# tsy935/eeg-gnn-ssl

Hardware: AMD Instinct MI355X
Metric: EEG clips/sec (60s, 19ch, K=2, 2-layer x64) fwd+bwd (higher is better)
Workload: dtype f32

## Files before the change

eeg_gnn_ssl_amd/csrc/api.cpp:

```cpp
#include <atomic>
#include <cmath>
#include <cstdarg>
#include <cstdio>
#include <cstring>

#include <string>
#include <vector>

#include "../../include/eeg_dcrnn.h"
#include "../../include/eeg_dcrnn_dev.h"
#include "../../include/eeg_dcrnn_prof.h"
#include "kernels_decoder.h"
#include "kernels_diffuse.h"
#include "kernels_eval.h"
#include "kernels_data.h"
#include "kernels_feat.h"
#include "kernels_gemm.h"
#include "kernels_gemm_bf.h"
#include "kernels_graph.h"
#include "kernels_head.h"
#include "kernels_pack.h"
#include "spec_common.h"
#include "spec_launch.h"
#include "kernels_tail.h"
// ... 320 lines not shown
    return w;
}


int cell_weight_grads(const eeg_layer_dims* d, const float* X, const float* planes, size_t x_stride, const float* Hprev,
                      const float* RHs, const float* dXW, const float* P, const float* hpl_in, const float* rpl_in,
                      size_t h_stride, float* hpl_ws, float* rpl_ws, float* part, const BwdWs& w, bool accumulate,
                      float* dWg, float* dWc, hipStream_t st, BtMap bt = BtMap(), const float* bias_part = nullptr,
                      float* dbg = nullptr, float* dbc = nullptr) {
    const int S = d->T * d->B, R = S * d->N, H = d->H, M = d->M, Fin = d->Fin, N = d->N;
    const int acc = accumulate ? 8 : 0;
    SegPtrs sx;
    for (int m = 0; m < kMaxM; ++m) sx.p[m] = m == 0 ? X : (m < M ? planes + (size_t)(m - 1) * x_stride : nullptr);
    float* part_g = part + (w.part_g - w.partial);
    float* part_c = part + (w.part_c - w.partial);
    if (gemm_tn(w.tx, w.cx, sx, dXW, 3 * H, 0, part, st, "gemm_tn_x", bt)) return 1;
    const float* hpl = hpl_in;
    size_t hs = h_stride;
    if (hpl == nullptr) {
        if (diffuse_fwd(Hprev, P, d->p_batched, S, d->B, N, H, M, hpl_ws, st)) return 1;
        hpl = hpl_ws;
        hs = (size_t)R * H;
    }
    SegPtrs sh;
    for (int m = 0; m < kMaxM; ++m) sh.p[m] = m == 0 ? Hprev : (m < M ? hpl + (size_t)(m - 1) * hs : nullptr);
    const float* rpl = rpl_in;
    size_t rs = h_stride;
    if (rpl == nullptr) {
        if (diffuse_fwd(RHs, P, d->p_batched, S, d->B, N, H, M, rpl_ws, st)) return 1;
        rpl = rpl_ws;
        rs = (size_t)R * H;
    }
    SegPtrs sr;
    for (int m = 0; m < kMaxM; ++m) sr.p[m] = m == 0 ? RHs : (m < M ? rpl + (size_t)(m - 1) * rs : nullptr);
    if (w.pair) {
        if (launch_tnq_pair(w.thg.q, w.thc.q, sh, sr, M, H, R, dXW, 3 * H, 0, 2 * H, part_g, 2 * H, H, part_c, st, "gemm_tn_h"))
            return fail("gemm_tnq_pair: launch failed");
    } else {
        if (gemm_tn(w.thg, w.chg, sh, dXW, 3 * H, 0, part_g, st, "gemm_tn_hg")) return 1;
        if (gemm_tn(w.thc, w.chc, sr, dXW, 3 * H, 2 * H, part_c, st, "gemm_tn_hc")) return 1;
    }
    ReduceJobs jobs;
    const int Ks[3] = {M * Fin, M * H, M * H}, Os[3] = {3 * H, 2 * H, H}, ns[3] = {w.tx.nsplit, w.thg.nsplit, w.thc.nsplit};
    const float* parts[3] = {part, part_g, part_c};
    int nblocks = 0;
    for (int j = 0; j < 3; ++j) {
        jobs.part[j] = parts[j]; jobs.nsplit[j] = ns[j]; jobs.K[j] = Ks[j]; jobs.O[j] = Os[j];
        jobs.nblocks[j] = ceil_div(Ks[j] * Os[j], 64);
        nblocks += jobs.nblocks[j];
    }
    jobs.bias_part = bias_part; jobs.bias_B = d->B; jobs.dbg = dbg; jobs.dbc = dbc;
    if (bias_part != nullptr) nblocks += ceil_div(3 * H, 16);
    EEG_LAUNCH_P("reduce_unpack", reduce_unpack3_kernel, dim3(nblocks), dim3(256), 256 * sizeof(float4), st, jobs, acc, Fin, H, M, dWg, dWc);
    return check_launch("reduce_unpack");
}

size_t xs_spec(const eeg_layer_dims* d) { return d->x_plane_stride > 0 ? (size_t)d->x_plane_stride : 0; }
int cell_weight_grads_spectral(const eeg_layer_dims* d, const float* Xh, size_t x_gs, const float* hh, size_t hh_gs, const float* rhh,
                               const float* dYh, float* part, const BwdWs& w, float* dWg, float* dWc, hipStream_t st,
                               const float* bias_part, float* dbg, float* dbc) {
    const int S = d->T * d->B, H = d->H, M = d->M, Fin = d->Fin, N = d->N, Sp = spec_rows(S);
    float* part_g = part + (w.part_g - w.partial);
    float* part_c = part + (w.part_c - w.partial);
    const SpecTnPlan& g = w.gs;
    if (spec_plan_error("weight gradients (spectral)", g.error)) return 1;
    if (g.fused) {
        if (launch_tnf(g, Xh, x_gs, Fin, hh, hh_gs, rhh, dYh, Sp, N, part, part_g, part_c, st, "gemm_tn_f")) return fail("gemm_tnf: launch failed");
    } else {
        if (launch_tng(g, Xh, x_gs, Fin, Sp, N, dYh, part, st, "gemm_tn_x")) return fail("gemm_tng: launch failed");
        if (launch_tng_pair(g, hh, hh_gs, rhh, Sp, N, dYh, part_g, part_c, st, "gemm_tn_h")) return fail("gemm_tng_pair: launch failed");
    }
    ReduceJobs jobs{};
    SpecFoldJobs sj{};
    sj.basis = d->spectral; sj.N = N;
    sj.j[0] = SpecFoldJob{part, g.spg_x, Fin, 3 * H, ceil_div(Fin * 3 * H, 64)};
    sj.j[1] = SpecFoldJob{part_g, g.spg_h, H, 2 * H, ceil_div(H * 2 * H, 64)};
    sj.j[2] = SpecFoldJob{part_c, g.spg_h, H, H, ceil_div(H * H, 64)};
    int nblocks = sj.j[0].nblocks + sj.j[1].nblocks + sj.j[2].nblocks;
    jobs.bias_part = bias_part; jobs.bias_B = d->B; jobs.dbg = dbg; jobs.dbc = dbc;
    if (bias_part != nullptr) nblocks += ceil_div(3 * H, 16);
    const int ns_max = N * (g.spg_x > g.spg_h ? g.spg_x : g.spg_h);
    const size_t fold_lds = spec_fold_lds_bytes(M, ns_max);
    EEG_SET_MAX_LDS(reduce_unpack3s_kernel, fold_lds);
    EEG_LAUNCH_P("reduce_unpack", reduce_unpack3s_kernel, dim3(nblocks), dim3(256), fold_lds, st, jobs, sj, 0, Fin, H, M, dWg, dWc);
    return check_launch("reduce_unpack (spectral)");
}

int colsum_rows_per_chunk(int R) { int rpc = ceil_div(R, 512); return rpc < 64 ? 64 : rpc; }
size_t colsum_ws(int R, int C) { return (size_t)ceil_div(R, colsum_rows_per_chunk(R)) * C; }
int colsum(const float* A, int R, int C, int split, float* ws, float* out0, float* out1, hipStream_t st) {
    const int rpc = colsum_rows_per_chunk(R), nchunk = ceil_div(R, rpc);
    if (C % 4 == 0 && C <= 1024) {
        const int nrs = 256 / (C / 4);
        EEG_LAUNCH_P("reduce_bias", colsum_partial4_kernel, dim3(nchunk), dim3(256), (size_t)nrs * C * sizeof(float), st, A, R, C, rpc, ws);
    } else {
        EEG_LAUNCH_P("reduce_bias", colsum_partial_kernel, dim3(nchunk, ceil_div(C, 128)), dim3(256), 256 * sizeof(float), st, A, R, C, rpc, ws);
    }
    if (check_launch("colsum_partial")) return 1;
    EEG_LAUNCH_P("reduce_bias", colsum_final_kernel, dim3(ceil_div(C, 128)), dim3(128), 0, st, ws, nchunk, C, split, out0, out1);
    return check_launch("colsum_final");
}

struct DecLayout {
    size_t xin, proj_pack, proj_bias, hd, saved_total;
    size_t planes[8], hext[8], rs[8], us[8], cs[8], rhs[8], hpl[8], rpl[8];
    size_t dxw[8], dbias[8], dotot, da, dhn, z, partial, projt_pack, colsum, bwd_total;
    TnCall cp;
    TnPlan tp;
    BwdWs lw[8];
    eeg_layer_dims ld[8];
};
size_t align64(size_t v) { return (v + 63) / 64 * 64; }
DecLayout dec_layout(const eeg_decoder_dims* d) {
    DecLayout y;
    const size_t state = (size_t)d->B * d->N * d->H, R = (size_t)d->T * d->B * d->N;
    const int nct_o = ceil_div(d->Dout, 16), nct_h = ceil_div(d->H, 16);
    size_t o = 0;
    y.xin = o;       o += align64(R * d->Dout);
    y.proj_pack = o; o += align64((size_t)(d->H / 4) * nct_o * 64);
    y.proj_bias = o; o += align64((size_t)nct_o * 16);
    for (int l = 0; l < d->L; ++l) {
        const int fin = l == 0 ? d->Dout : d->H;
        y.ld[l] = eeg_layer_dims{d->T, d->B, d->N, d->H, fin, d->M, d->act, d->p_batched, 0, 0, 0};
        y.planes[l] = o; if (l == 0) o += align64((size_t)(d->M - 1) * R * fin);
        y.hext[l] = o;   o += align64((size_t)(d->T + 1) * state);
        y.rs[l] = o;     o += align64((size_t)d->T * state);
        y.us[l] = o;     o += align64((size_t)d->T * state);
        y.cs[l] = o;     o += align64((size_t)d->T * state);
        y.rhs[l] = o;    o += align64((size_t)d->T * state);
        y.hpl[l] = o;    o += align64((size_t)(d->M - 1) * (d->T + 1) * state);
        y.rpl[l] = o;    o += align64((size_t)(d->M - 1) * (d->T + 1) * state);
    }
    y.hd = d->dropout_p > 0.f ? o : y.hext[d->L - 1] + state;
    if (d->dropout_p > 0.f) o += align64((size_t)d->T * state);
    y.saved_total = o;
    o = 0;
    size_t part = 0;
    for (int l = 0; l < d->L; ++l) {
        y.lw[l] = bwd_ws(&y.ld[l], 0);
        y.dxw[l] = o; o += align64(R * 3 * d->H);
        const size_t pl = y.lw[l].total - y.lw[l].partial;
        part = pl > part ? pl : part;
    }
    for (int l = 0; l < d->L; ++l) { y.dbias[l] = o; o += (size_t)d->T * d->B * 3 * d->H; }
    o = align64(o);
    y.dotot = o;  o += align64(R * d->Dout);
    y.da = o;     o += align64(state);
    y.dhn = o;    o += align64(2 * (size_t)d->L * state);
    y.z = o;      o += align64((size_t)d->B * d->N * d->M * (d->Dout > d->H ? d->Dout : d->H));
    y.cp = tn_call(1, d->Dout, (int)R, d->H);
    y.tp = gemm_tn_plan(y.cp);
    const size_t pp = (size_t)y.tp.nsplit * d->Dout * d->H;
    part = pp > part ? pp : part;
    y.partial = o; o += align64(part);
    y.projt_pack = o; o += align64((size_t)(d->Dout / 4) * nct_h * 64);
    const size_t c1 = colsum_ws((int)R, d->Dout), c2 = colsum_ws(d->L * d->T * d->B, 3 * d->H);
    y.colsum = o; o += align64(c1 > c2 ? c1 : c2);
    y.bwd_total = o;
    return y;
}
int check_dropout_p(const char* who, float p) {
    if (!(p >= 0.f && p <= 1.f)) return fail("%s: dropout probability has to be between 0 and 1, but got %g", who, p);
    return 0;
}
int check_decoder_dims(const eeg_decoder_dims* d) {
    if (d->L < 1 || d->L > 8) return fail("decoder: num_rnn_layers=%d unsupported (1..8)", d->L);
    if (d->T < 1 || d->B < 1) return fail("decoder: empty sequence/batch (T=%d, B=%d)", d->T, d->B);
// ... 1306 lines not shown
```

eeg_gnn_ssl_amd/csrc/kernels_pack.h:

```cpp
#pragma once
#include "common.h"
#include "nnq_order.h"
#include "spec_common.h"
#include "pack_cell.h"

namespace eeg {

__global__ void pack_cell_kernel(const float* __restrict__ Wg, const float* __restrict__ bg,
                                 const float* __restrict__ Wc, const float* __restrict__ bc,
                                 float* __restrict__ out, CellPack p) {
    pack_cell_body(Wg, bg, Wc, bc, out, p, (int)blockIdx.x, (int)gridDim.x);
}

__global__ void pack_dense_kernel(const float* __restrict__ W, int F, int M, int O, float* __restrict__ out) {
    const size_t total = (size_t)F * M * O;
    const int nct = O / 16;
    for (size_t e = (size_t)blockIdx.x * blockDim.x + threadIdx.x; e < total; e += (size_t)gridDim.x * blockDim.x) {
        const int lane = e & 63, ct = (e >> 6) % nct, ks = (e >> 6) / nct;
        const int k = 4 * ks + (lane >> 4), j = 16 * ct + (lane & 15);
        const int m = k / F, f = k % F;
        out[e] = W[((size_t)f * M + m) * O + j];
    }
}

__global__ void pack_dense_t_kernel(const float* __restrict__ W, int F, int M, int O, float* __restrict__ out) {
    const int nct = round_up(M * F, 16) / 16;
    const size_t total = (size_t)(O / 4) * nct * 64;
    for (size_t e = (size_t)blockIdx.x * blockDim.x + threadIdx.x; e < total; e += (size_t)gridDim.x * blockDim.x) {
        const int lane = e & 63, ct = (e >> 6) % nct, ks = (e >> 6) / nct;
        const int o = 4 * ks + (lane >> 4), j = 16 * ct + (lane & 15);
        float v = 0.f;
        if (j < M * F) v = W[((size_t)(j % F) * M + j / F) * O + o];
        out[e] = v;
    }
}

__global__ void pack_linear_kernel(const float* __restrict__ W, int Out, int In, int transposed, float* __restrict__ out) {
    const int K = transposed ? In : Out, O = transposed ? Out : In;
    const int nct = (O + 15) / 16;
    const size_t total = (size_t)(K / 4) * nct * 64;
    for (size_t e = (size_t)blockIdx.x * blockDim.x + threadIdx.x; e < total; e += (size_t)gridDim.x * blockDim.x) {
        const int lane = e & 63, ct = (e >> 6) % nct, ks = (e >> 6) / nct;
        const int k = 4 * ks + (lane >> 4), j = 16 * ct + (lane & 15);
        float v = 0.f;
        if (j < O) v = transposed ? W[(size_t)j * In + k] : W[(size_t)k * In + j];
        out[e] = v;
    }
}

__device__ __forceinline__ void reduce_unpack_block(int block, const float* __restrict__ part, int nsplit, int K, int O,
                                                    int kind_flags, int Fin, int H, int M,
                                                    float* __restrict__ dWg, float* __restrict__ dWc) {
    EEG_DYN_SMEM(sm);
    float4 (*red)[16] = reinterpret_cast<float4 (*)[16]>(sm);
    const size_t total = (size_t)K * O;
    const int g = threadIdx.x >> 4, q = threadIdx.x & 15;
    const size_t idx4 = ((size_t)block * 16 + q) * 4;
    float4 a = make_float4(0.f, 0.f, 0.f, 0.f);
    if (idx4 < total) {
        for (int sp = g; sp < nsplit; sp += 16) {
            const float4 v = *reinterpret_cast<const float4*>(part + (size_t)sp * total + idx4);
            a.x += v.x; a.y += v.y; a.z += v.z; a.w += v.w;
        }
    }
    red[g][q] = a;
    __syncthreads();
    if (g != 0 || idx4 >= total) return;
    float4 sum = red[0][q];
#pragma unroll
    for (int u = 1; u < 16; ++u) {
        const float4 v = red[u][q];
        sum.x += v.x; sum.y += v.y; sum.z += v.z; sum.w += v.w;
    }
    const float sv[4] = {sum.x, sum.y, sum.z, sum.w};
    const bool accumulate = (kind_flags & 8) != 0;
    const int kind = kind_flags & 7;
#pragma unroll
    for (int e = 0; e < 4; ++e) {
        const size_t idx = idx4 + e;
        const int k = idx / O, o = idx % O;
        float* dst;
        if (kind == 0) {
            const int m = k / Fin, f = k % Fin;
            dst = o < 2 * H ? &dWg[((size_t)f * M + m) * (2 * H) + o] : &dWc[((size_t)f * M + m) * H + (o - 2 * H)];
        } else if (kind == 1) {
            dst = &dWg[((size_t)(Fin + k % H) * M + k / H) * (2 * H) + o];
        } else if (kind == 3) {
            dst = &dWg[idx];
        } else if (kind == 4) {
            dst = &dWg[((size_t)(k % Fin) * M + k / Fin) * O + o];
        } else {
            dst = &dWc[((size_t)(Fin + k % H) * M + k / H) * H + o];
        }
        *dst = accumulate ? *dst + sv[e] : sv[e];
    }
}
__global__ __launch_bounds__(256) void reduce_unpack_kernel(const float* __restrict__ part, int nsplit, int K, int O,
                                                            int kind_flags, int Fin, int H, int M,
                                                            float* __restrict__ dWg, float* __restrict__ dWc) {
    reduce_unpack_block(blockIdx.x, part, nsplit, K, O, kind_flags, Fin, H, M, dWg, dWc);
}
__device__ __forceinline__ void reduce_bias_block(int blk, float* sm, const float* __restrict__ part, int B, int H,
                                                  float* __restrict__ dbg, float* __restrict__ dbc) {
    const int c = threadIdx.x & 15, q = threadIdx.x >> 4;
    const int j = blk * 16 + c;
    float s = 0.f;
    if (j < 3 * H)
        for (int b = q; b < B; b += 16) s += part[(size_t)b * 3 * H + j];
    sm[q * 16 + c] = s;
    __syncthreads();
    if (q == 0 && j < 3 * H) {
        float t = 0.f;
        for (int i = 0; i < 16; ++i) t += sm[i * 16 + c];
        if (j < 2 * H) dbg[j] = t; else dbc[j - 2 * H] = t;
    }
}
struct ReduceJobs {
    const float* part[3]; int nsplit[3]; int K[3]; int O[3]; int nblocks[3];
    const float* bias_part; int bias_B; float* dbg; float* dbc;
};
__global__ __launch_bounds__(256) void reduce_unpack3_kernel(ReduceJobs jobs, int flags, int Fin, int H, int M,
                                                             float* __restrict__ dWg, float* __restrict__ dWc) {
    int b = blockIdx.x, j = 0;
    if (b >= jobs.nblocks[0]) { b -= jobs.nblocks[0]; j = 1; }
    if (j == 1 && b >= jobs.nblocks[1]) { b -= jobs.nblocks[1]; j = 2; }
    if (j == 2 && b >= jobs.nblocks[2]) {
        EEG_DYN_SMEM(sm);
        reduce_bias_block(b - jobs.nblocks[2], sm, jobs.bias_part, jobs.bias_B, H, jobs.dbg, jobs.dbc);
        return;
    }
    reduce_unpack_block(b, jobs.part[j], jobs.nsplit[j], jobs.K[j], jobs.O[j], j | flags, Fin, H, M, dWg, dWc);
}

__global__ __launch_bounds__(256) void reduce_unpack3s_kernel(ReduceJobs jobs, SpecFoldJobs sj, int flags, int Fin, int H, int M,
                                                              float* __restrict__ dWg, float* __restrict__ dWc) {
    int b = blockIdx.x;
#pragma unroll
    for (int k = 0; k < 3; ++k) {
        if (sj.j[k].part == nullptr) continue;
        if (b < sj.j[k].nblocks) {
            spec_fold_block(b, sj.j[k], k, sj.basis, sj.N, (flags & 8) != 0 ? 1 : 0, Fin, H, M, dWg, dWc);
            return;
        }
        b -= sj.j[k].nblocks;
    }
#pragma unroll
    for (int j = 1; j < 3; ++j) {
        if (sj.j[j].part != nullptr) continue;
        if (b < jobs.nblocks[j]) {
            reduce_unpack_block(b, jobs.part[j], jobs.nsplit[j], jobs.K[j], jobs.O[j], j | flags, Fin, H, M, dWg, dWc);
            return;
        }
        b -= jobs.nblocks[j];
    }
    EEG_DYN_SMEM(sm);
    reduce_bias_block(b, sm, jobs.bias_part, jobs.bias_B, H, jobs.dbg, jobs.dbc);
}

__global__ void colsum_partial_kernel(const float* __restrict__ A, int R, int C, int rpc, float* __restrict__ partial) {
    EEG_DYN_SMEM(sm);
    const int c = threadIdx.x & 127, q = threadIdx.x >> 7;
    const int col = blockIdx.y * 128 + c;
    const int r0 = blockIdx.x * rpc, r1 = (r0 + rpc < R) ? r0 + rpc : R;
    float a0 = 0.f, a1 = 0.f, a2 = 0.f, a3 = 0.f;
    if (col < C) {
        int r = r0 + q;
        for (; r + 6 < r1; r += 8) {
            a0 += A[(size_t)r * C + col];
            a1 += A[(size_t)(r + 2) * C + col];
            a2 += A[(size_t)(r + 4) * C + col];
            a3 += A[(size_t)(r + 6) * C + col];
        }
        for (; r < r1; r += 2) a0 += A[(size_t)r * C + col];
    }
    sm[q * 128 + c] = (a0 + a1) + (a2 + a3);
    __syncthreads();
    if (q == 0 && col < C) partial[(size_t)blockIdx.x * C + col] = sm[c] + sm[128 + c];
}
__global__ __launch_bounds__(256) void colsum_partial4_kernel(const float* __restrict__ A, int R, int C, int rpc,
                                                              float* __restrict__ partial) {
    EEG_DYN_SMEM(sm);
    const int c4n = C / 4, nrs = 256 / c4n;
    const int cq = threadIdx.x % c4n, q = threadIdx.x / c4n;
    const int r0 = blockIdx.x * rpc, r1 = (r0 + rpc < R) ? r0 + rpc : R;
    f32x4 a0 = {0.f, 0.f, 0.f, 0.f}, a1 = a0, a2 = a0, a3 = a0;
    if (q < nrs) {
        const float* p = A + 4 * cq;
        int r = r0 + q;
        for (; r + 3 * nrs < r1; r += 4 * nrs) {
            a0 += ld4(p + (size_t)r * C);
            a1 += ld4(p + (size_t)(r + nrs) * C);
            a2 += ld4(p + (size_t)(r + 2 * nrs) * C);
            a3 += ld4(p + (size_t)(r + 3 * nrs) * C);
        }
        for (; r < r1; r += nrs) a0 += ld4(p + (size_t)r * C);
        st4(sm + q * C + 4 * cq, (a0 + a1) + (a2 + a3));
    }
    __syncthreads();
    for (int col = threadIdx.x; col < C; col += 256) {
        float s = 0.f;
        for (int i = 0; i < nrs; ++i) s += sm[i * C + col];
        partial[(size_t)blockIdx.x * C + col] = s;
    }
}
__global__ void colsum_final_kernel(const float* __restrict__ partial, int nchunk, int C, int split,
                                    float* __restrict__ out0, float* __restrict__ out1) {
    const int col = blockIdx.x * blockDim.x + threadIdx.x;
    if (col >= C) return;
    float a0 = 0.f, a1 = 0.f, a2 = 0.f, a3 = 0.f;
    int i = 0;
    for (; i + 4 <= nchunk; i += 4) {
        a0 += partial[(size_t)i * C + col];
        a1 += partial[(size_t)(i + 1) * C + col];
        a2 += partial[(size_t)(i + 2) * C + col];
        a3 += partial[(size_t)(i + 3) * C + col];
    }
    for (; i < nchunk; ++i) a0 += partial[(size_t)i * C + col];
    const float s = (a0 + a1) + (a2 + a3);
// ... 50 lines not shown
```

eeg_gnn_ssl_amd/csrc/kernels_spectral.h:

```cpp
#pragma once
#include "spec_common.h"
#include "spec_launch.h"

namespace eeg {

__global__ __launch_bounds__(256) void spectral_basis_kernel(const float* __restrict__ S, int N, float* __restrict__ out) {
    EEG_DYN_SMEM(sm);
    double* A = reinterpret_cast<double*>(sm);
    double* V = A + 32 * 32;
    double* cs = V + 32 * 32;
    int* pq = reinterpret_cast<int*>(cs + 32);
    double* red = reinterpret_cast<double*>(pq + 32);
    const int tid = threadIdx.x;
    const int NP = (N + 1) & ~1, NH = NP / 2;
    for (int e = tid; e < 32 * 32; e += 256) {
        const int i = e >> 5, j = e & 31;
        A[e] = (i < N && j < N) ? 0.5 * ((double)S[i * N + j] + (double)S[j * N + i]) : 0.0;
        V[e] = i == j ? 1.0 : 0.0;
    }
    __syncthreads();
    for (int sweep = 0; sweep < kSpecSweeps; ++sweep) {
        for (int r = 0; r < NP - 1; ++r) {
            if (tid < NH) {
                int p = tid == 0 ? NP - 1 : (r + tid) % (NP - 1);
// ... 38 lines not shown
    }
    for (int e = tid; e < N * N; e += 256) out[e] = (float)V[(e / N) * 32 + (e % N)];
    for (int e = tid; e < kSpecTc; e += 256) {
        const int m = e >> 5, i = e & 31;
        double t = 0.0;
        if (i < N) {
            const double lam = A[i * 32 + i];
            double t0 = 1.0, t1 = lam;
            t = m == 0 ? t0 : t1;
            for (int k = 2; k <= m; ++k) { t = 2.0 * lam * t1 - t0; t0 = t1; t1 = t; }
        }
        out[N * N + e] = (float)t;
    }
    double rmax = 0.0, omax = 0.0, smax = 0.0;
    for (int e = tid; e < N * N; e += 256) {
        const int i = e / N, j = e % N;
        double rec = 0.0;
        for (int k = 0; k < N; ++k) rec += V[i * 32 + k] * A[k * 32 + k] * V[j * 32 + k];
        rmax = fmax(rmax, fabs((double)S[e] - rec));
        if (i != j) omax = fmax(omax, fabs(A[i * 32 + j]));
        smax = fmax(smax, fabs((double)S[e]));
    }
    for (int which = 0; which < 3; ++which) {
        __syncthreads();
        red[tid] = which == 0 ? rmax : (which == 1 ? omax : smax);
        __syncthreads();
        if (tid == 0) {
            double m = 0.0;
            for (int i = 0; i < 256; ++i) m = fmax(m, red[i]);
            out[N * N + kSpecTc + which] = (float)m;
        }
    }
    if (tid >= 3 && tid < kSpecInfo) out[N * N + kSpecTc + tid] = 0.f;
    if (tid < 32) {
        double c = 0.0;
        if (tid < N)
            for (int n = 0; n < N; ++n) c += V[n * 32 + tid];
        out[N * N + kSpecTc + kSpecInfo + tid] = (float)c;
    }
}

__device__ __forceinline__ void pack_spectral_body(const float* __restrict__ Wg, const float* __restrict__ Wc, const float* __restrict__ basis,
                                                   float* __restrict__ out, const SpecPack& p, int bid, int nb) {
    const int Fin = p.Fin, H = p.H, M = p.M, N = p.N;
    const float* tc = basis + N * N;
    const NnqOrder ox = make_nnq_order(1, Fin), ot = make_nnq_order(1, 3 * H);
    const size_t stride = (size_t)nb * blockDim.x;
    for (size_t idx = (size_t)bid * blockDim.x + threadIdx.x; idx < p.total; idx += stride) {
        if (idx >= p.sxr) {
            const size_t e0 = idx - p.sxr;
            const int i = (int)(e0 / p.sxr_stride), e = (int)(e0 - (size_t)i * p.sxr_stride), f = e / (3 * H), o = e - f * 3 * H;
            float v = 0.f;
            if (f < Fin)
                for (int m = 0; m < M; ++m) {
                    const float w = o < 2 * H ? Wg[((size_t)f * M + m) * (2 * H) + o] : Wc[((size_t)f * M + m) * H + (o - 2 * H)];
                    v = fmaf(tc[m * 32 + i], w, v);
                }
            out[idx] = v;
            continue;
        }
        const bool tr = idx >= p.sxtq;
        const size_t bs = tr ? p.sxtq_stride : p.sxq_stride, e0 = idx - (tr ? p.sxtq : p.sxq);
        const int i = (int)(e0 / bs);
        const size_t e = e0 - (size_t)i * bs;
        const int s4 = e & 3, lane = (e >> 2) & 63, nct = tr ? p.nct_t : p.nct_x;
        const int ct = (int)((e >> 8) % nct), c = (int)((e >> 8) / nct), j = 16 * ct + (lane & 15);
        const int k = nnq_k_of(tr ? ot : ox, c, lane >> 4, s4);
        float v = 0.f;
        if (k >= 0) {
            const int f = tr ? j : k, o = tr ? k : j;
            if (f < Fin) {
                for (int m = 0; m < M; ++m) {
                    const float w = o < 2 * H ? Wg[((size_t)f * M + m) * (2 * H) + o] : Wc[((size_t)f * M + m) * H + (o - 2 * H)];
                    v = fmaf(tc[m * 32 + i], w, v);
                }
            }
        }
        out[idx] = v;
    }
}
__global__ void pack_spectral_kernel(const float* __restrict__ Wg, const float* __restrict__ Wc, const float* __restrict__ basis,
                                     float* __restrict__ out, SpecPack p) {
    pack_spectral_body(Wg, Wc, basis, out, p, (int)blockIdx.x, (int)gridDim.x);
}

__device__ __forceinline__ size_t spec_sample(size_t r, int map, int T, int B) { return map ? (r % B) * (size_t)T + r / B : r; }

template <int N>
__global__ __launch_bounds__(256) void spec_mix_in_kernel(const float* __restrict__ X, const float* __restrict__ basis, int S, int Sp,
                                                         int F, int map, int T, int B, float* __restrict__ Xh) {
    const int F4 = F / 4, SPW = blockDim.x / F4;
    const int tl = threadIdx.x / F4, c4 = threadIdx.x % F4;
    if (tl >= SPW) return;
    const float* __restrict__ U = basis;
    const float4* X4 = reinterpret_cast<const float4*>(X);
    float4* O4 = reinterpret_cast<float4*>(Xh);
    for (int r = blockIdx.x * SPW + tl; r < Sp; r += gridDim.x * SPW) {
        if (r >= S) {
#pragma unroll
            for (int i = 0; i < N; ++i) O4[((size_t)i * Sp + r) * F4 + c4] = make_float4(0.f, 0.f, 0.f, 0.f);
            continue;
        }
        const size_t s = spec_sample((size_t)r, map, T, B);
        float4 x[N];
#pragma unroll
        for (int n = 0; n < N; ++n) x[n] = X4[(s * N + n) * F4 + c4];
#pragma unroll
        for (int i = 0; i < N; ++i) {
            float4 a = make_float4(0.f, 0.f, 0.f, 0.f);
#pragma unroll
            for (int n = 0; n < N; ++n) {
                const float u = U[n * N + i];
                a.x = fmaf(u, x[n].x, a.x);
                a.y = fmaf(u, x[n].y, a.y);
                a.z = fmaf(u, x[n].z, a.z);
                a.w = fmaf(u, x[n].w, a.w);
            }
            O4[((size_t)i * Sp + r) * F4 + c4] = a;
        }
    }
}

template <int N>
__global__ __launch_bounds__(256) void spec_mix_out_kernel(const float* __restrict__ Yh, const float* __restrict__ basis,
                                                          const float* __restrict__ bias, int S, int Sp, int F, int map, int T, int B,
                                                          float* __restrict__ Y) {
    const int F4 = F / 4, SPW = blockDim.x / F4;
    const int tl = threadIdx.x / F4, c4 = threadIdx.x % F4;
    if (tl >= SPW) return;
    const float* __restrict__ U = basis;
    const float4* I4 = reinterpret_cast<const float4*>(Yh);
    float4* O4 = reinterpret_cast<float4*>(Y);
    float4 bv = make_float4(0.f, 0.f, 0.f, 0.f);
    if (bias != nullptr) bv = reinterpret_cast<const float4*>(bias)[c4];
    for (int r = blockIdx.x * SPW + tl; r < S; r += gridDim.x * SPW) {
        const size_t s = spec_sample((size_t)r, map, T, B);
        float4 y[N];
#pragma unroll
        for (int i = 0; i < N; ++i) y[i] = I4[((size_t)i * Sp + r) * F4 + c4];
#pragma unroll
        for (int j = 0; j < N; ++j) {
            float4 a = bv;
#pragma unroll
            for (int i = 0; i < N; ++i) {
                const float u = U[j * N + i];
                a.x = fmaf(u, y[i].x, a.x);
                a.y = fmaf(u, y[i].y, a.y);
                a.z = fmaf(u, y[i].z, a.z);
                a.w = fmaf(u, y[i].w, a.w);
            }
            O4[(s * N + j) * F4 + c4] = a;
        }
    }
}

template <int DIR, int KS>
__global__ __launch_bounds__(256) void spec_mix_mfma_kernel(const float* __restrict__ in, const float* __restrict__ basis,
                                                           const float* __restrict__ bias, int N, int S, int Sp, int F, int map, int T,
                                                           int B, float* __restrict__ out) {
    const int lane = threadIdx.x & 63, hh = lane >> 5, l32 = lane & 31;
    const int gw = (int)blockIdx.x * 4 + wave_uniform((int)threadIdx.x >> 6), nw = (int)gridDim.x * 4;
    float a[KS];
#pragma unroll
    for (int ks = 0; ks < KS; ++ks) {
        const int k = 2 * ks + hh;
        a[ks] = (k < N && l32 < N) ? (DIR == 0 ? basis[k * N + l32] : basis[l32 * N + k]) : 0.f;
// ... 78 lines not shown
```

eeg_gnn_ssl_amd/csrc/spec_common.h:

```cpp
#pragma once
#include "common.h"
#include "nnq_order.h"

namespace eeg {

constexpr int kSpecTc = kMaxM * 32, kSpecInfo = 32, kSpecCsum = 32;
__host__ __device__ constexpr int spec_basis_floats(int N) { return N * N + kSpecTc + kSpecInfo + kSpecCsum; }
__host__ __device__ constexpr int spec_csum_offset(int N) { return N * N + kSpecTc + kSpecInfo; }
__host__ __device__ constexpr int spec_rows(int S) { return round_up(S, 16); }
constexpr int kSpecSweeps = 12;

struct SpecPack {
    int Fin, H, M, N;
    int nch_x, nct_x, nch_t, nct_t;
    size_t sxq, sxq_stride, sxtq, sxtq_stride, sxr, sxr_stride, total;
};
__host__ __device__ inline SpecPack make_spec_pack(int Fin, int H, int M, int N) {
    SpecPack p;
    p.Fin = Fin; p.H = H; p.M = M; p.N = N;
    p.nch_x = make_nnq_order(1, Fin).nch; p.nct_x = 3 * H / 16;
    p.nch_t = make_nnq_order(1, 3 * H).nch; p.nct_t = round_up(Fin, 16) / 16;
    p.sxq_stride = (size_t)p.nch_x * p.nct_x * 256;
    p.sxtq_stride = (size_t)p.nch_t * p.nct_t * 256;
    p.sxq = 0;
    p.sxtq = p.sxq + p.sxq_stride * N;
    p.sxr = p.sxtq + p.sxtq_stride * N;
    p.sxr_stride = (size_t)round_up(Fin, 8) * 3 * H;
    p.total = p.sxr + p.sxr_stride * N;
    return p;
}
struct SpecFoldJob {
    const float* part;
    int spg, K, O, nblocks;
};
struct SpecFoldJobs {
    SpecFoldJob j[3];
    const float* basis;
    int N;
};
__host__ __device__ inline size_t spec_fold_lds_bytes(int M, int nsplit_max) { return 256 * 16 + (size_t)M * nsplit_max * sizeof(float); }
template <int MM>
__device__ __forceinline__ void spec_fold_block_m(int block, const SpecFoldJob& jb, int kind, const float* __restrict__ basis, int N,
                                                   int acc_flag, int Fin, int H, int M, float* __restrict__ dWg, float* __restrict__ dWc) {
    EEG_DYN_SMEM(sm);
    float4 (*red)[16] = reinterpret_cast<float4 (*)[16]>(sm);
    float* tcl = sm + 256 * 4;
    const int O = jb.O;
    const size_t total = (size_t)jb.K * O;
    const int g = threadIdx.x >> 4, q = threadIdx.x & 15;
    const size_t idx4 = ((size_t)block * 16 + q) * 4;
    const float* tc = basis + N * N;
    const int nsplit = N * jb.spg;
    for (int e = threadIdx.x; e < M * nsplit; e += 256) {
        const int m = e / nsplit, sp = e - m * nsplit;
        tcl[e] = tc[m * 32 + sp / jb.spg];
    }
    __syncthreads();
    float4 a[MM];
#pragma unroll
    for (int m = 0; m < MM; ++m) a[m] = make_float4(0.f, 0.f, 0.f, 0.f);
    if (idx4 < total) {
        constexpr int UN = 8;
        for (int base = g; base < nsplit; base += 16 * UN) {
            float4 v[UN];
#pragma unroll
            for (int u = 0; u < UN; ++u) {
                const int sp = base + 16 * u;
                v[u] = sp < nsplit ? *reinterpret_cast<const float4*>(jb.part + (size_t)sp * total + idx4) : make_float4(0.f, 0.f, 0.f, 0.f);
            }
#pragma unroll
            for (int u = 0; u < UN; ++u) {
                const int sp = base + 16 * u < nsplit ? base + 16 * u : 0;
#pragma unroll
                for (int m = 0; m < MM; ++m) {
                    if (m < M) {
                        const float t = tcl[m * nsplit + sp];
                        a[m].x = fmaf(t, v[u].x, a[m].x); a[m].y = fmaf(t, v[u].y, a[m].y);
                        a[m].z = fmaf(t, v[u].z, a[m].z); a[m].w = fmaf(t, v[u].w, a[m].w);
                    }
                }
            }
        }
    }
#pragma unroll
    for (int m = 0; m < MM; ++m) {
        if (m >= M) break;
        __syncthreads();
        red[g][q] = a[m];
        __syncthreads();
        if (g == 0 && idx4 < total) {
            float4 sum = red[0][q];
#pragma unroll
            for (int u = 1; u < 16; ++u) {
                const float4 v = red[u][q];
                sum.x += v.x; sum.y += v.y; sum.z += v.z; sum.w += v.w;
            }
            const float sv[4] = {sum.x, sum.y, sum.z, sum.w};
#pragma unroll
            for (int e = 0; e < 4; ++e) {
                const size_t idx = idx4 + e;
                const int f = (int)(idx / O), o = (int)(idx % O);
                float* dst;
                if (kind == 0) dst = o < 2 * H ? &dWg[((size_t)f * M + m) * (2 * H) + o] : &dWc[((size_t)f * M + m) * H + (o - 2 * H)];
                else if (kind == 1) dst = &dWg[((size_t)(Fin + f) * M + m) * (2 * H) + o];
                else dst = &dWc[((size_t)(Fin + f) * M + m) * H + o];
                *dst = acc_flag ? *dst + sv[e] : sv[e];
            }
        }
    }
}
__device__ __forceinline__ void spec_fold_block(int block, const SpecFoldJob& jb, int kind, const float* __restrict__ basis, int N,
                                                int acc_flag, int Fin, int H, int M, float* __restrict__ dWg, float* __restrict__ dWc) {
    if (M <= 4) spec_fold_block_m<4>(block, jb, kind, basis, N, acc_flag, Fin, H, M, dWg, dWc);
    else spec_fold_block_m<kMaxM>(block, jb, kind, basis, N, acc_flag, Fin, H, M, dWg, dWc);
}

}
```

eeg_gnn_ssl_amd/csrc/spec_inst.cpp:

```cpp
#include "kernels_gemm_g.h"
#include "kernels_gemm_f.h"
#include "kernels_spectral.h"
#include "pack_cell.h"
#include "spec_launch.h"
#include "prof.h"

namespace eeg {

constexpr int kMaxPackJobs = 8;
struct PackJob {
    const float *Wg, *bg, *Wc, *bc, *basis;
    float* out;
    int spectral;
    CellPack cp;
    SpecPack sp;
};
struct PackJobs { PackJob j[kMaxPackJobs]; };
__global__ void pack_cells_kernel(PackJobs jobs) {
    const PackJob& jb = jobs.j[blockIdx.y];
    if (jb.spectral) pack_spectral_body(jb.Wg, jb.Wc, jb.basis, jb.out, jb.sp, (int)blockIdx.x, (int)gridDim.x);
    else pack_cell_body(jb.Wg, jb.bg, jb.Wc, jb.bc, jb.out, jb.cp, (int)blockIdx.x, (int)gridDim.x);
}


size_t spec_pack_floats(int Fin, int H, int M, int N) { return make_spec_pack(Fin, H, M, N).total; }

int launch_spec_basis(const float* S, int N, float* basis, hipStream_t st) {
    EEG_SET_MAX_LDS(spectral_basis_kernel, kSpecBasisLds);
    EEG_LAUNCH_P("spec_basis", spectral_basis_kernel, dim3(1), dim3(256), kSpecBasisLds, st, S, N, basis);
    return hipGetLastError() == hipSuccess ? 0 : 2;
}

int launch_spec_pack(const float* Wg, const float* Wc, const float* basis, int Fin, int H, int M, int N, float* spack, hipStream_t st) {
    const SpecPack p = make_spec_pack(Fin, H, M, N);
    EEG_LAUNCH_P("pack_cell", pack_spectral_kernel, dim3(1024), dim3(256), 0, st, Wg, Wc, basis, spack, p);
    return hipGetLastError() == hipSuccess ? 0 : 2;
}

int launch_pack_cells(int n_cells, const float* const* Wg, const float* const* bg, const float* const* Wc, const float* const* bc,
                      const int* Fin, int H, int M, float* const* packs, const float* basis, int N, float* const* spacks, hipStream_t st) {
    PackJobs jobs{};
    int n = 0;
    for (int c = 0; c < n_cells; ++c) {
        if (n + (spacks != nullptr ? 2 : 1) > kMaxPackJobs) return 1;
        PackJob& a = jobs.j[n++];
        a.Wg = Wg[c]; a.bg = bg[c]; a.Wc = Wc[c]; a.bc = bc[c]; a.basis = nullptr; a.out = packs[c]; a.spectral = 0;
        a.cp = make_cell_pack(Fin[c], H, M);
        if (spacks != nullptr) {
            PackJob& b = jobs.j[n++];
            b.Wg = Wg[c]; b.bg = nullptr; b.Wc = Wc[c]; b.bc = nullptr; b.basis = basis; b.out = spacks[c]; b.spectral = 1;
            b.sp = make_spec_pack(Fin[c], H, M, N);
        }
    }
    EEG_LAUNCH_P("pack_cell", pack_cells_kernel, dim3(256, n), dim3(256), 0, st, jobs);
    return hipGetLastError() == hipSuccess ? 0 : 2;
}

int launch_spec_mix(const SpecMixPlan& p, const float* in, const float* basis, int N, int T, int B, int F, int bm, float* out,
                    hipStream_t st, const char* tag) {
    const float* bias = nullptr;
    const dim3 grid(p.grid), block(p.block);
#define EEG_MIX_MFMA(DIR, KS) EEG_LAUNCH_P(tag, (spec_mix_mfma_kernel<DIR, KS>), grid, block, p.lds, st, in, basis, bias, N, p.S, p.Sp, F, bm, T, B, out)
    if (p.kind == SpecMixKind::Mfma) {
        if (p.ks == 10) { if (p.to_nodes) EEG_MIX_MFMA(0, 10); else EEG_MIX_MFMA(1, 10); }
        else { if (p.to_nodes) EEG_MIX_MFMA(0, 16); else EEG_MIX_MFMA(1, 16); }
    } else if (p.kind == SpecMixKind::Valu19) {
        if (p.to_nodes) EEG_LAUNCH_P(tag, spec_mix_in_kernel<19>, grid, block, p.lds, st, in, basis, p.S, p.Sp, F, bm, T, B, out);
        else EEG_LAUNCH_P(tag, spec_mix_out_kernel<19>, grid, block, p.lds, st, in, basis, bias, p.S, p.Sp, F, bm, T, B, out);
    } else {
        EEG_LAUNCH_P(tag, spec_mix_generic_kernel, grid, block, p.lds, st, in, basis, bias, N, p.S, p.Sp, F, bm, T, B, p.to_nodes, out);
    }
#undef EEG_MIX_MFMA
    return hipGetLastError() == hipSuccess ? 0 : 2;
}

int launch_spec_zero_rows(float* Xh, int N, int S, int Sp, int F, hipStream_t st) {
    if (Sp <= S) return 0;
    EEG_LAUNCH_P("zero", spec_zero_pad_kernel, dim3(ceil_div(N * (Sp - S) * F, 256)), dim3(256), 0, st, Xh, N, S, Sp, F);
    return hipGetLastError() == hipSuccess ? 0 : 2;
}

namespace {
template <int KQ, bool SWZ>
void launch_nnf_one(const SpecNnPlan& p, const float* A, size_t ags, int K, int Sp, int G, const float* Wr, size_t wstride, float* C, hipStream_t st,
                    const char* tag, const float* bias, const float* gscale) {
    EEG_SET_MAX_LDS((gemm_nnf_kernel<KQ, SWZ>), p.lds);
    EEG_LAUNCH_P(tag, (gemm_nnf_kernel<KQ, SWZ>), dim3(p.grid), dim3(p.block), p.lds, st, A, (long long)ags, K, Sp, G, Wr, (unsigned)wstride, C, bias, gscale);
}
template <int NJ>
void launch_nng_one(const SpecNnPlan& p, const float* A, size_t ags, int F, int Sp, int G, const float* Wq, size_t wstride, float* C, hipStream_t st,
                    const char* tag, const float* bias, const float* gscale) {
    EEG_SET_MAX_LDS((gemm_nng_kernel<NJ, 2>), p.lds);
    EEG_LAUNCH_P(tag, (gemm_nng_kernel<NJ, 2>), dim3(p.grid), dim3(p.block), p.lds, st, A, (unsigned)ags, F, Sp, G, Wq, (unsigned)wstride, C, 64 * NJ, bias, gscale);
}
}
int launch_spec_nn(const SpecNnPlan& p, const float* A, size_t a_gstride, int K, int Sp, int G, const float* W, size_t wstride, float* C,
                   hipStream_t st, const char* tag, const float* bias, const float* gscale) {
    const size_t ags = a_gstride != 0 ? a_gstride : (size_t)Sp * K;
#define EEG_NNF(KQ, SWZ) launch_nnf_one<KQ, SWZ>(p, A, ags, K, Sp, G, W, wstride, C, st, tag, bias, gscale)
    if (p.kind == SpecNnKind::Regs) {
        switch (p.kq) {
            case 8: EEG_NNF(8, true); break;
            case 13: EEG_NNF(13, false); break;
            case 9: EEG_NNF(9, false); break;
            case 5: EEG_NNF(5, false); break;
            case 2: EEG_NNF(2, false); break;
            default: return 1;
        }
    } else if (p.nj == 3) {
        launch_nng_one<3>(p, A, ags, K, Sp, G, W, wstride, C, st, tag, bias, gscale);
    } else if (p.nj == 1) {
        launch_nng_one<1>(p, A, ags, K, Sp, G, W, wstride, C, st, tag, bias, gscale);
    } else {
        return 1;
    }
#undef EEG_NNF
    return hipGetLastError() == hipSuccess ? 0 : 2;
}

namespace {
template <int KT, bool PLANAR>
void launch_tng_one(const SpecTnPlan& p, const float* A, int F, int Sp, int G, const float* dY, float* partial, hipStream_t st, const char* tag,
                    long long skew) {
    constexpr int RC = kSpecTngRc, OT = kSpecTngOt;
    SegPtrs segs;
    for (int m = 0; m < kMaxM; ++m) segs.p[m] = m == 0 ? A : nullptr;
    EEG_SET_MAX_LDS((gemm_tnq_grouped_kernel<KT, OT, RC, PLANAR>), p.lds_x);
    EEG_LAUNCH_P(tag, (gemm_tnq_grouped_kernel<KT, OT, RC, PLANAR>), dim3(p.grid_x, p.grid_y), dim3(p.block), p.lds_x, st, segs, F, Sp, G, p.spg_x, dY,
                 192, 0, 192, partial, p.rps_x, skew);
}
template <int FXT>
void launch_tnf_one(const SpecTnPlan& p, const float* Xh, size_t xgs, int Fin, const float* Hh, size_t hgs, const float* RHh, const float* dY,
                    int Sp, float* part_x, float* part_g, float* part_c, hipStream_t st, const char* tag) {
    EEG_SET_MAX_LDS((gemm_tnf_kernel<FXT>), p.lds_x);
    EEG_LAUNCH_P(tag, (gemm_tnf_kernel<FXT>), dim3(p.grid_x, p.grid_y), dim3(p.block), p.lds_x, st, Xh, (long long)xgs, Fin, Hh, (long long)hgs, RHh, dY,
                 Sp, p.spg_x, p.rps_x, part_x, part_g, part_c);
}
// ... 51 lines not shown
```

Baseline: 138,100.

## Widen spectral fold reduction to 512 threads and reshape spectral weight packing

The spectral weight-gradient fold kernel now runs with 512 threads per block. It reduces per-m partials with wave shuffles and does a single LDS pass, replacing the repeated syncthreads/LDS reductions done once per m. The weight packing launch gets a flattened grid sized to each job's real work. Spectral packing uses a new body where each thread loads its M weights once and writes all N frequency outputs. Together these target the backward-pass reduction and weight-pack overheads, at the cost of more LDS per block and a larger block size that may lower occupancy.

```diff
diff --git a/eeg_gnn_ssl_amd/csrc/api.cpp b/eeg_gnn_ssl_amd/csrc/api.cpp
--- a/eeg_gnn_ssl_amd/csrc/api.cpp
+++ b/eeg_gnn_ssl_amd/csrc/api.cpp
@@ -426,7 +426,7 @@
     const int ns_max = N * (g.spg_x > g.spg_h ? g.spg_x : g.spg_h);
     const size_t fold_lds = spec_fold_lds_bytes(M, ns_max);
     EEG_SET_MAX_LDS(reduce_unpack3s_kernel, fold_lds);
-    EEG_LAUNCH_P("reduce_unpack", reduce_unpack3s_kernel, dim3(nblocks), dim3(256), fold_lds, st, jobs, sj, 0, Fin, H, M, dWg, dWc);
+    EEG_LAUNCH_P("reduce_unpack", reduce_unpack3s_kernel, dim3(nblocks), dim3(kSpecFoldThreads), fold_lds, st, jobs, sj, 0, Fin, H, M, dWg, dWc);
     return check_launch("reduce_unpack (spectral)");
 }
 
diff --git a/eeg_gnn_ssl_amd/csrc/kernels_pack.h b/eeg_gnn_ssl_amd/csrc/kernels_pack.h
--- a/eeg_gnn_ssl_amd/csrc/kernels_pack.h
+++ b/eeg_gnn_ssl_amd/csrc/kernels_pack.h
@@ -57,13 +57,13 @@
     const int g = threadIdx.x >> 4, q = threadIdx.x & 15;
     const size_t idx4 = ((size_t)block * 16 + q) * 4;
     float4 a = make_float4(0.f, 0.f, 0.f, 0.f);
-    if (idx4 < total) {
+    if (g < 16 && idx4 < total) {
         for (int sp = g; sp < nsplit; sp += 16) {
             const float4 v = *reinterpret_cast<const float4*>(part + (size_t)sp * total + idx4);
             a.x += v.x; a.y += v.y; a.z += v.z; a.w += v.w;
         }
     }
-    red[g][q] = a;
+    if (g < 16) red[g][q] = a;
     __syncthreads();
     if (g != 0 || idx4 >= total) return;
     float4 sum = red[0][q];
@@ -105,9 +105,9 @@
     const int c = threadIdx.x & 15, q = threadIdx.x >> 4;
     const int j = blk * 16 + c;
     float s = 0.f;
-    if (j < 3 * H)
+    if (q < 16 && j < 3 * H)
         for (int b = q; b < B; b += 16) s += part[(size_t)b * 3 * H + j];
-    sm[q * 16 + c] = s;
+    if (q < 16) sm[q * 16 + c] = s;
     __syncthreads();
     if (q == 0 && j < 3 * H) {
         float t = 0.f;
@@ -132,8 +132,8 @@
     reduce_unpack_block(b, jobs.part[j], jobs.nsplit[j], jobs.K[j], jobs.O[j], j | flags, Fin, H, M, dWg, dWc);
 }
 
-__global__ __launch_bounds__(256) void reduce_unpack3s_kernel(ReduceJobs jobs, SpecFoldJobs sj, int flags, int Fin, int H, int M,
-                                                              float* __restrict__ dWg, float* __restrict__ dWc) {
+__global__ __launch_bounds__(kSpecFoldThreads, 4) void reduce_unpack3s_kernel(ReduceJobs jobs, SpecFoldJobs sj, int flags, int Fin, int H, int M,
+                                                                           float* __restrict__ dWg, float* __restrict__ dWc) {
     int b = blockIdx.x;
 #pragma unroll
     for (int k = 0; k < 3; ++k) {
diff --git a/eeg_gnn_ssl_amd/csrc/kernels_spectral.h b/eeg_gnn_ssl_amd/csrc/kernels_spectral.h
--- a/eeg_gnn_ssl_amd/csrc/kernels_spectral.h
+++ b/eeg_gnn_ssl_amd/csrc/kernels_spectral.h
@@ -144,6 +144,47 @@
 __global__ void pack_spectral_kernel(const float* __restrict__ Wg, const float* __restrict__ Wc, const float* __restrict__ basis,
                                      float* __restrict__ out, SpecPack p) {
     pack_spectral_body(Wg, Wc, basis, out, p, (int)blockIdx.x, (int)gridDim.x);
+}
+
+__host__ __device__ inline size_t spec_pack_units(const SpecPack& p) { return p.sxq_stride + p.sxtq_stride + p.sxr_stride; }
+__device__ __forceinline__ void pack_spectral_freq_body(const float* __restrict__ Wg, const float* __restrict__ Wc, const float* __restrict__ basis,
+                                                        float* __restrict__ out, const SpecPack& p, int bid) {
+    const int Fin = p.Fin, H = p.H, M = p.M, N = p.N;
+    const float* tc = basis + N * N;
+    const size_t u = (size_t)bid * blockDim.x + threadIdx.x;
+    if (u >= spec_pack_units(p)) return;
+    size_t base, bs, e;
+    int f, o;
+    bool on;
+    if (u >= p.sxq_stride + p.sxtq_stride) {
+        e = u - (p.sxq_stride + p.sxtq_stride);
+        f = (int)(e / (3 * H)); o = (int)(e - (size_t)f * 3 * H);
+        on = f < Fin;
+        base = p.sxr; bs = p.sxr_stride;
+    } else {
+        const bool tr = u >= p.sxq_stride;
+        e = u - (tr ? p.sxq_stride : 0);
+        const int s4 = e & 3, lane = (e >> 2) & 63, nct = tr ? p.nct_t : p.nct_x;
+        const int ct = (int)((e >> 8) % nct), c = (int)((e >> 8) / nct), j = 16 * ct + (lane & 15);
+        const int k = nnq_k_of(tr ? make_nnq_order(1, 3 * H) : make_nnq_order(1, Fin), c, lane >> 4, s4);
+        f = tr ? j : k; o = tr ? k : j;
+        on = k >= 0 && f < Fin;
+        base = tr ? p.sxtq : p.sxq; bs = tr ? p.sxtq_stride : p.sxq_stride;
+    }
+    float w[kMaxM];
+#pragma unroll
+    for (int m = 0; m < kMaxM; ++m) {
+        w[m] = 0.f;
+        if (on && m < M) w[m] = o < 2 * H ? Wg[((size_t)f * M + m) * (2 * H) + o] : Wc[((size_t)f * M + m) * H + (o - 2 * H)];
+    }
+    float* dst = out + base + e;
+    for (int i = 0; i < N; ++i) {
+        float v = 0.f;
+#pragma unroll
+        for (int m = 0; m < kMaxM; ++m)
+            if (m < M) v = fmaf(tc[m * 32 + i], w[m], v);
+        dst[(size_t)i * bs] = on ? v : 0.f;
+    }
 }
 
 __device__ __forceinline__ size_t spec_sample(size_t r, int map, int T, int B) { return map ? (r % B) * (size_t)T + r / B : r; }
diff --git a/eeg_gnn_ssl_amd/csrc/spec_common.h b/eeg_gnn_ssl_amd/csrc/spec_common.h
--- a/eeg_gnn_ssl_amd/csrc/spec_common.h
+++ b/eeg_gnn_ssl_amd/csrc/spec_common.h
@@ -29,6 +29,7 @@
     p.total = p.sxr + p.sxr_stride * N;
     return p;
 }
+constexpr int kSpecFoldThreads = 512;
 struct SpecFoldJob {
     const float* part;
     int spg, K, O, nblocks;
@@ -38,20 +39,25 @@
     const float* basis;
     int N;
 };
-__host__ __device__ inline size_t spec_fold_lds_bytes(int M, int nsplit_max) { return 256 * 16 + (size_t)M * nsplit_max * sizeof(float); }
+__host__ __device__ inline size_t spec_fold_red_floats(int M) { return (size_t)M * (kSpecFoldThreads / 64) * 64; }
+__host__ __device__ inline size_t spec_fold_lds_bytes(int M, int nsplit_max) {
+    const size_t b = (spec_fold_red_floats(M) + (size_t)M * nsplit_max) * sizeof(float);
+    return b < 256 * 16 ? 256 * 16 : b;
+}
 template <int MM>
 __device__ __forceinline__ void spec_fold_block_m(int block, const SpecFoldJob& jb, int kind, const float* __restrict__ basis, int N,
                                                    int acc_flag, int Fin, int H, int M, float* __restrict__ dWg, float* __restrict__ dWc) {
     EEG_DYN_SMEM(sm);
-    float4 (*red)[16] = reinterpret_cast<float4 (*)[16]>(sm);
-    float* tcl = sm + 256 * 4;
+    constexpr int G = kSpecFoldThreads / 16, NW = kSpecFoldThreads / 64;
+    float4* red = reinterpret_cast<float4*>(sm);
+    float* tcl = sm + spec_fold_red_floats(M);
     const int O = jb.O;
     const size_t total = (size_t)jb.K * O;
-    const int g = threadIdx.x >> 4, q = threadIdx.x & 15;
+    const int g = threadIdx.x >> 4, q = threadIdx.x & 15, wv = threadIdx.x >> 6;
     const size_t idx4 = ((size_t)block * 16 + q) * 4;
     const float* tc = basis + N * N;
     const int nsplit = N * jb.spg;
-    for (int e = threadIdx.x; e < M * nsplit; e += 256) {
+    for (int e = threadIdx.x; e < M * nsplit; e += kSpecFoldThreads) {
         const int m = e / nsplit, sp = e - m * nsplit;
         tcl[e] = tc[m * 32 + sp / jb.spg];
     }
@@ -60,17 +66,17 @@
 #pragma unroll
     for (int m = 0; m < MM; ++m) a[m] = make_float4(0.f, 0.f, 0.f, 0.f);
     if (idx4 < total) {
-        constexpr int UN = 8;
-        for (int base = g; base < nsplit; base += 16 * UN) {
+        constexpr int UN = MM <= 4 ? 8 : 4;
+        for (int base = g; base < nsplit; base += G * UN) {
             float4 v[UN];
 #pragma unroll
             for (int u = 0; u < UN; ++u) {
-                const int sp = base + 16 * u;
+                const int sp = base + G * u;
                 v[u] = sp < nsplit ? *reinterpret_cast<const float4*>(jb.part + (size_t)sp * total + idx4) : make_float4(0.f, 0.f, 0.f, 0.f);
             }
 #pragma unroll
             for (int u = 0; u < UN; ++u) {
-                const int sp = base + 16 * u < nsplit ? base + 16 * u : 0;
+                const int sp = base + G * u < nsplit ? base + G * u : 0;
 #pragma unroll
                 for (int m = 0; m < MM; ++m) {
                     if (m < M) {
@@ -85,28 +91,32 @@
 #pragma unroll
     for (int m = 0; m < MM; ++m) {
         if (m >= M) break;
-        __syncthreads();
-        red[g][q] = a[m];
-        __syncthreads();
-        if (g == 0 && idx4 < total) {
-            float4 sum = red[0][q];
 #pragma unroll
-            for (int u = 1; u < 16; ++u) {
-                const float4 v = red[u][q];
-                sum.x += v.x; sum.y += v.y; sum.z += v.z; sum.w += v.w;
-            }
-            const float sv[4] = {sum.x, sum.y, sum.z, sum.w};
+        for (int x = 16; x <= 32; x *= 2) {
+            a[m].x += __shfl_xor(a[m].x, x); a[m].y += __shfl_xor(a[m].y, x);
+            a[m].z += __shfl_xor(a[m].z, x); a[m].w += __shfl_xor(a[m].w, x);
+        }
+        if ((threadIdx.x & 63) < 16) red[(m * NW + wv) * 16 + q] = a[m];
+    }
+    __syncthreads();
+    const int m = threadIdx.x >> 4;
+    if (m >= M || idx4 >= total) return;
+    float4 sum = red[(m * NW) * 16 + q];
 #pragma unroll
-            for (int e = 0; e < 4; ++e) {
-                const size_t idx = idx4 + e;
-                const int f = (int)(idx / O), o = (int)(idx % O);
-                float* dst;
-                if (kind == 0) dst = o < 2 * H ? &dWg[((size_t)f * M + m) * (2 * H) + o] : &dWc[((size_t)f * M + m) * H + (o - 2 * H)];
-                else if (kind == 1) dst = &dWg[((size_t)(Fin + f) * M + m) * (2 * H) + o];
-                else dst = &dWc[((size_t)(Fin + f) * M + m) * H + o];
-                *dst = acc_flag ? *dst + sv[e] : sv[e];
-            }
-        }
+    for (int u = 1; u < NW; ++u) {
+        const float4 v = red[(m * NW + u) * 16 + q];
+        sum.x += v.x; sum.y += v.y; sum.z += v.z; sum.w += v.w;
+    }
+    const float sv[4] = {sum.x, sum.y, sum.z, sum.w};
+#pragma unroll
+    for (int e = 0; e < 4; ++e) {
+        const size_t idx = idx4 + e;
+        const int f = (int)(idx / O), o = (int)(idx % O);
+        float* dst;
+        if (kind == 0) dst = o < 2 * H ? &dWg[((size_t)f * M + m) * (2 * H) + o] : &dWc[((size_t)f * M + m) * H + (o - 2 * H)];
+        else if (kind == 1) dst = &dWg[((size_t)(Fin + f) * M + m) * (2 * H) + o];
+        else dst = &dWc[((size_t)(Fin + f) * M + m) * H + o];
+        *dst = acc_flag ? *dst + sv[e] : sv[e];
     }
 }
 __device__ __forceinline__ void spec_fold_block(int block, const SpecFoldJob& jb, int kind, const float* __restrict__ basis, int N,
diff --git a/eeg_gnn_ssl_amd/csrc/spec_inst.cpp b/eeg_gnn_ssl_amd/csrc/spec_inst.cpp
--- a/eeg_gnn_ssl_amd/csrc/spec_inst.cpp
+++ b/eeg_gnn_ssl_amd/csrc/spec_inst.cpp
@@ -15,11 +15,14 @@
     CellPack cp;
     SpecPack sp;
 };
-struct PackJobs { PackJob j[kMaxPackJobs]; };
-__global__ void pack_cells_kernel(PackJobs jobs) {
-    const PackJob& jb = jobs.j[blockIdx.y];
-    if (jb.spectral) pack_spectral_body(jb.Wg, jb.Wc, jb.basis, jb.out, jb.sp, (int)blockIdx.x, (int)gridDim.x);
-    else pack_cell_body(jb.Wg, jb.bg, jb.Wc, jb.bc, jb.out, jb.cp, (int)blockIdx.x, (int)gridDim.x);
+struct PackJobs { PackJob j[kMaxPackJobs]; int first[kMaxPackJobs + 1]; int n; };
+__global__ __launch_bounds__(256) void pack_cells_kernel(PackJobs jobs) {
+    int k = 0;
+    while (k + 1 < jobs.n && (int)blockIdx.x >= jobs.first[k + 1]) ++k;
+    const PackJob& jb = jobs.j[k];
+    const int bid = (int)blockIdx.x - jobs.first[k], nb = jobs.first[k + 1] - jobs.first[k];
+    if (jb.spectral) pack_spectral_freq_body(jb.Wg, jb.Wc, jb.basis, jb.out, jb.sp, bid);
+    else pack_cell_body(jb.Wg, jb.bg, jb.Wc, jb.bc, jb.out, jb.cp, bid, nb);
 }
 
 
@@ -43,16 +46,21 @@
     int n = 0;
     for (int c = 0; c < n_cells; ++c) {
         if (n + (spacks != nullptr ? 2 : 1) > kMaxPackJobs) return 1;
-        PackJob& a = jobs.j[n++];
+        PackJob& a = jobs.j[n];
         a.Wg = Wg[c]; a.bg = bg[c]; a.Wc = Wc[c]; a.bc = bc[c]; a.basis = nullptr; a.out = packs[c]; a.spectral = 0;
         a.cp = make_cell_pack(Fin[c], H, M);
+        jobs.first[n + 1] = jobs.first[n] + (int)((a.cp.total + 255) / 256);
+        ++n;
         if (spacks != nullptr) {
-            PackJob& b = jobs.j[n++];
+            PackJob& b = jobs.j[n];
             b.Wg = Wg[c]; b.bg = nullptr; b.Wc = Wc[c]; b.bc = nullptr; b.basis = basis; b.out = spacks[c]; b.spectral = 1;
             b.sp = make_spec_pack(Fin[c], H, M, N);
+            jobs.first[n + 1] = jobs.first[n] + (int)((spec_pack_units(b.sp) + 255) / 256);
+            ++n;
         }
     }
-    EEG_LAUNCH_P("pack_cell", pack_cells_kernel, dim3(256, n), dim3(256), 0, st, jobs);
+    jobs.n = n;
+    EEG_LAUNCH_P("pack_cell", pack_cells_kernel, dim3(jobs.first[n]), dim3(256), 0, st, jobs);
     return hipGetLastError() == hipSuccess ? 0 : 2;
 }
 
```

Result: no change. 138,900 (median of 6 runs) (+0.6%).
